# CycloneBoy/pdf_table

Hardware: AMD Instinct MI355X
Metric: pages/s (higher is better)
Workload: dtype bf16

## Files before the change

pdf_table_amd/csrc/rec_kernels.hip:

```cpp
#include <math.h>

#include "common.h"

namespace PT_FMT_NS {

typedef __attribute__((ext_vector_type(8))) __bf16 bf16x8;
typedef __attribute__((ext_vector_type(16))) float f32x16;
typedef __attribute__((ext_vector_type(4))) uint32_t u32x4;
typedef __attribute__((ext_vector_type(2))) uint32_t u32x2;

__device__ __forceinline__ float rbf2f(uint32_t bits16) { return a16_to_f32(bits16); }
__device__ __forceinline__ uint32_t rf2bf(float f) { return f32_to_a16(f); }

__global__ __launch_bounds__(256) void rec_warp_kernel(const uint8_t* __restrict__ pages, int ph, int pw,
                                                        const pt_rec_line* __restrict__ lines, int n_lines,
                                                        const long long* __restrict__ pix_off, uint8_t* __restrict__ crops) {
  a16_kernel_enter();
  const int li = blockIdx.y;
  if (li >= n_lines) return;
  const pt_rec_line L = lines[li];
  const int cw = L.crop_w, chh = L.crop_h;
  const long long npx = (long long)cw * chh;
  uint8_t* dst = crops + pix_off[li] * 3;
  const uint8_t* src = pages + (size_t)L.page * ph * pw * 3;
// ... 999 lines not shown
    __syncthreads();
    if (tid == 0) __hip_atomic_store(fl + member, s + 1, __ATOMIC_RELAXED, __HIP_MEMORY_SCOPE_AGENT);
#pragma unroll
    for (int i = 0; i < 2 * MI; ++i) {
      const int idx = tio + i * 256, m = idx >> 3, pc = idx & 7;
      const int line = line0 + m;
      if (line < B) *reinterpret_cast<u32x4*>(hout + ((size_t)line * T + t) * 512 + dir * 256 + member * 64 + pc * 8) = pv[i];
    }
  }
}

template <int MI>
static int launch_lstm_cluster(const bf16_t* gx, const bf16_t* whh, bf16_t* hout, int B, int T, int max_cl, bf16_t* hx, int* flags,
                               int* err, hipStream_t s) {
  constexpr int CLL = 64 * MI;
  constexpr int SMEM = 131072 + CLL * 72 * 2;
  static bool attr_done = false;
  if (!attr_done) {
    PT_HIP_CHECK(hipFuncSetAttribute(reinterpret_cast<const void*>(&lstm_cluster_kernel<MI>), hipFuncAttributeMaxDynamicSharedMemorySize, SMEM));
    attr_done = true;
  }
  const int nlaunch = (B + max_cl * CLL - 1) / (max_cl * CLL);
  const int per = (((B + nlaunch - 1) / nlaunch) + CLL - 1) / CLL * CLL;
  for (int b0 = 0; b0 < B; b0 += per) {
    const int nb = (B - b0) < per ? (B - b0) : per;
    const int ncl = (nb + CLL - 1) / CLL;
    PT_HIP_CHECK(hipMemsetAsync(flags, 0, (size_t)(2 * max_cl * 4) * sizeof(int), s));
    hipLaunchKernelGGL(lstm_cluster_kernel<MI>, dim3(((ncl + 7) / 8) * 32, 2), dim3(256), SMEM, s, gx + (size_t)b0 * T * 2048, whh,
                       hout + (size_t)b0 * T * 512, nb, T, ncl, hx, flags, err);
  }
  return PT_OK;
}

template <int MI, int NW>
__global__ __launch_bounds__(64 * NW, 1) void lstm_cluster8_x3_kernel(const bf16_t* __restrict__ gx, const bf16_t* __restrict__ whh,
                                                                   bf16_t* __restrict__ hout, int B, int T, int ncl,
                                                                   unsigned long long* __restrict__ hx, int* __restrict__ flags,
                                                                   int* __restrict__ err) {
  a16_kernel_enter();
  constexpr int CLL = 32 * NW * MI, NTILE = NW * MI, NTHR = 64 * NW;
  extern __shared__ __attribute__((aligned(16))) char lsm[];
  char* wl = lsm;
  constexpr int SROW = 32;
  bf16_t* stage = reinterpret_cast<bf16_t*>(lsm + 131072) + (threadIdx.x >> 6) * (2 * 32 * SROW);
  const int tid = threadIdx.x, lane = tid & 63, wave = tid >> 6;
  const int lx = lane & 31, q = lane >> 5;
  const int L = blockIdx.x, dir = blockIdx.y;
  const int member = (L >> 3) & 7, cl = (L >> 6) * 8 + (L & 7);
  if (cl >= ncl) return;
  const int line0 = cl * CLL;
  {
    for (int i = tid; i < 2 * 64 * 64; i += NTHR) {
      const int pl = i >> 12, rec = (i >> 6) & 63, ln = i & 63;
      const bf16_t* src = whh + (size_t)pl * 2 * 1024 * 256 + (size_t)dir * 1024 * 256 + (size_t)(member >> 1) * 65536 +
                          (size_t)(rec * 2 + (member & 1)) * 512 + ln * 8;
      *reinterpret_cast<u32x4*>(wl + (size_t)pl * 65536 + rec * 1024 + ln * 16) = *reinterpret_cast<const u32x4*>(src);
    }
  }
  constexpr size_t XBUF = (size_t)NTILE * 16 * 2 * 64 * 2;
  unsigned long long* hxc = hx + (size_t)(dir * ncl + cl) * 2 * XBUF;
  int* fl = flags + (dir * ncl + cl) * 8;
  float c[MI][16];
#pragma unroll
  for (int mi = 0; mi < MI; ++mi)
#pragma unroll
    for (int r = 0; r < 16; ++r) c[mi][r] = 0.f;
// ... 142 lines not shown
    PT_HIP_CHECK(hipMalloc(&e->lstm_scratch8, need));
    e->lstm_scratch8_cap = need;
  }
  unsigned long long* hx = reinterpret_cast<unsigned long long*>(e->lstm_scratch8);
  int* flags = reinterpret_cast<int*>(reinterpret_cast<char*>(e->lstm_scratch8) + (size_t)2 * max_cl * 2 * xbuf);
  int* err = nullptr;
  PT_HIP_CHECK(hipHostGetDevicePointer(reinterpret_cast<void**>(&err), e->lstm_err, 0));
  const int nlaunch = (B + max_cl * CLL - 1) / (max_cl * CLL);
  const int per = (((B + nlaunch - 1) / nlaunch) + CLL - 1) / CLL * CLL;
  for (int b0 = 0; b0 < B; b0 += per) {
    const int nb = (B - b0) < per ? (B - b0) : per;
    const int ncl = (nb + CLL - 1) / CLL;
    PT_HIP_CHECK(hipMemsetAsync(flags, 0, (size_t)(2 * max_cl * 8) * sizeof(int), s));
    hipLaunchKernelGGL((lstm_cluster8_x3_kernel<MI, NW>), dim3(((ncl + 7) / 8) * 64, 2), dim3(64 * NW), SMEM, s, gx + (size_t)b0 * T * 4096, whh,
                       hout + (size_t)b0 * T * 1024, nb, T, ncl, hx, flags, err);
  }
  return PT_OK;
}

int pt_launch_lstm(pt_engine* e, const bf16_t* gx, const bf16_t* whh, bf16_t* hout, int B, int T, int split, hipStream_t s) {
  if (B <= 0) return PT_OK;
  dim3 grid((B + 31) / 32, 2);
  static int ng2 = -1;
  if (ng2 < 0) {
    const char* ev = getenv("PT_LSTM_NG");
    ng2 = ev ? (atoi(ev) == 2) : 1;
  }
  static int use_dma = -1;
  if (use_dma < 0) {
    const char* ev = getenv("PT_LSTM_DMA");
    use_dma = ev ? atoi(ev) : 0;
  }
  if (!split && e->lstm_cluster) {
    if (!e->lstm_scratch) {
      e->lstm_max_cl = e->num_cu / 8 < 1 ? 1 : e->num_cu / 8;
      PT_HIP_CHECK(hipMalloc(&e->lstm_scratch, (size_t)2 * e->lstm_max_cl * 2 * CLL_MAX * 256 * sizeof(bf16_t) + (size_t)2 * e->lstm_max_cl * 4 * sizeof(int) + 256));
      PT_HIP_CHECK(hipHostMalloc(reinterpret_cast<void**>(&e->lstm_err), sizeof(int), hipHostMallocMapped));
      *e->lstm_err = 0;
    }
    void* scratch = e->lstm_scratch;
    int* h_err = e->lstm_err;
    const int max_cl = e->lstm_max_cl;
    if (*h_err) {
      *h_err = 0;
      e->lstm_cluster = 0;
      pt_set_error("lstm_cluster_kernel: a workgroup waited > 2^22 polls for its peers -- the launch was not co-resident "
                   "(GPU shared with another process or stream?).  Results of that call are invalid; this engine now uses "
                   "the streaming LSTM kernel: run the batch again");
      return PT_ERR_HIP;
    }
    bf16_t* hx = reinterpret_cast<bf16_t*>(scratch);
    int* flags = reinterpret_cast<int*>(reinterpret_cast<char*>(scratch) + (size_t)2 * max_cl * 2 * CLL_MAX * 256 * sizeof(bf16_t));
    int* err = nullptr;
    PT_HIP_CHECK(hipHostGetDevicePointer(reinterpret_cast<void**>(&err), h_err, 0));
    const char* ev = getenv("PT_LSTM_MI");
    const int force = ev ? atoi(ev) : 0;
    const int n2 = (B + max_cl * 128 - 1) / (max_cl * 128), n3 = (B + max_cl * 192 - 1) / (max_cl * 192);
    const bool mi3 = force == 3 || (force != 2 && n3 < n2);
    const int rc = mi3 ? launch_lstm_cluster<3>(gx, whh, hout, B, T, max_cl, hx, flags, err, s)
                       : launch_lstm_cluster<2>(gx, whh, hout, B, T, max_cl, hx, flags, err, s);
    if (rc != PT_OK) return rc;
  } else if (split == 1 && e->lstm_cluster && !(getenv("PT_LSTM_CLUSTER_X3") && atoi(getenv("PT_LSTM_CLUSTER_X3")) == 0)) {
    if (!e->lstm_err) {
      PT_HIP_CHECK(hipHostMalloc(reinterpret_cast<void**>(&e->lstm_err), sizeof(int), hipHostMallocMapped));
      *e->lstm_err = 0;
    }
    if (*e->lstm_err) {
      *e->lstm_err = 0;
      e->lstm_cluster = 0;
      pt_set_error("lstm_cluster8_x3_kernel: a workgroup waited > 2^22 polls for its peers -- the launch was not co-resident "
                   "(GPU shared with another process or stream?).  Results of that call are invalid; this engine now uses "
                   "the streaming LSTM kernel: run the batch again");
      return PT_ERR_HIP;
    }
    const int max_cl = e->num_cu / 16 < 1 ? 1 : e->num_cu / 16;
    const char* ev = getenv("PT_LSTM_MI");
    const int force = ev ? atoi(ev) : 0;
    const char* wv = getenv("PT_LSTM_X3_WAVES");
    int rc;
    if (wv && atoi(wv) == 4) {
      const int n2 = (B + max_cl * 256 - 1) / (max_cl * 256), n3 = (B + max_cl * 384 - 1) / (max_cl * 384);
      const bool mi3 = force == 3 || (force != 2 && n3 < n2);
      rc = mi3 ? launch_lstm_cluster8_x3<3, 4>(e, gx, whh, hout, B, T, s) : launch_lstm_cluster8_x3<2, 4>(e, gx, whh, hout, B, T, s);
    } else {
      const int n1 = (B + max_cl * 256 - 1) / (max_cl * 256), n2 = (B + max_cl * 512 - 1) / (max_cl * 512);
      const bool mi2 = force == 2 || (force != 1 && n2 < n1);
      rc = mi2 ? launch_lstm_cluster8_x3<2, 8>(e, gx, whh, hout, B, T, s) : launch_lstm_cluster8_x3<1, 8>(e, gx, whh, hout, B, T, s);
    }
    if (rc != PT_OK) return rc;
  } else if (split) {
    if (ng2)
      hipLaunchKernelGGL((lstm_dir_kernel<1, 2>), dim3((B + 63) / 64, 2), dim3(512), 0, s, gx, whh, hout, B, T);
    else
// ... 758 lines not shown
```

include/pdftable_hip.h:

```cpp
#ifndef PDFTABLE_HIP_H
#define PDFTABLE_HIP_H

#include <stddef.h>
#include <stdint.h>

#ifdef __cplusplus
extern "C" {
#endif

#define PT_OK 0
#define PT_ERR_INVALID 1
#define PT_ERR_HIP 2
#define PT_ERR_STATE 3
#define PT_ERR_FORMAT 4

typedef struct pt_engine pt_engine;
typedef void* pt_stream;

int pt_engine_create(int device_id, pt_engine** out);
void pt_engine_destroy(pt_engine* e);
const char* pt_last_error(void);
int pt_abi_version(void);
int pt_engine_check(pt_engine* e);
int pt_engine_set_lstm_cluster(pt_engine* e, int on);
// ... 133 lines not shown
  double minv[6];
  int32_t page, x0, y0, crop_w, crop_h, reserved;
} pt_tsr_table;

int pt_tsr_preprocess(pt_engine* e, const uint8_t* d_pages_rgb, int n_pages, int ph, int pw, const pt_tsr_table* d_tables,
                      int n, int inp_h, int inp_w, int bgr, uint16_t* d_out_bf16, pt_stream stream);

#define PT_TSR_CS_SMALL 8
#define PT_TSR_CS_FEAT 256
int pt_tsr_forward_net(pt_engine* e, const uint16_t* d_input_bf16, int n, int H, int W, float* d_hm, float* d_st,
                       float* d_wh, float* d_ax, float* d_cr, float* d_reg, pt_stream stream);

int pt_tsr_forward_net_wireless(pt_engine* e, const uint16_t* d_input_bf16, int n, int H, int W, float* d_hm, float* d_st,
                                float* d_wh, float* d_ax, float* d_cr, float* d_reg, pt_stream stream);

#define PT_TSR_MAX_CELLS 3000
int pt_tsr_decode(pt_engine* e, const float* d_hm, const float* d_st, const float* d_wh, const float* d_ax,
                  const float* d_cr, const float* d_reg, int n, int h, int w, int wiz_rev, float vis_thresh,
                  int32_t* d_counts, float* d_dets, float* d_logi, pt_stream stream);

int pt_tsr_forward_decode(pt_engine* e, const uint16_t* d_input_bf16, int n, int in_h, int in_w, int wiz_rev,
                          float vis_thresh, int32_t* d_counts, float* d_dets, float* d_logi, pt_stream stream);

int pt_tsr_process(pt_engine* e, const float* d_logi, const float* d_dets, const int32_t* h_counts, int n_tables,
                   int use_2dpe, float* d_logic, float* d_stacked, pt_stream stream);

int pt_op_conv2d(pt_engine* e, const uint16_t* d_in, int B, int H, int W, int Cin, const uint16_t* d_w_tiled,
                 const float* d_bias, int N, int ks, int stride, uint16_t* d_out, int out_cstride, int out_coff,
                 int rep, int shuffle_cout, const uint16_t* d_res, int res_mode, int relu, int split, int out_lo_off,
                 pt_stream stream);
int pt_op_conv1x1_ex(pt_engine* e, const uint16_t* d_in, int B, int H, int W, int Cin, const uint16_t* d_w_tiled, const float* d_bias,
                     int N, uint16_t* d_out, float* d_out_f32, int out_cstride, int n_valid, const float* d_res_f32, int relu,
                     const int32_t* d_ylimit, pt_stream stream);

int pt_op_dcn(pt_engine* e, const uint16_t* d_in, const float* d_om, int B, int H, int W, int C, const uint16_t* d_w_tiled,
              const float* d_bias, int N, uint16_t* d_out, int relu, int split, pt_stream stream);

int pt_op_stem7x7(pt_engine* e, const uint16_t* d_in, int B, int H, int W, const uint16_t* d_w, const float* d_bias,
                  uint16_t* d_out, int split, pt_stream stream);
int pt_op_maxpool3x3s2(pt_engine* e, const uint16_t* d_in, int B, int H, int W, int C, uint16_t* d_out, int split,
                       pt_stream stream);
int pt_op_db_head_final(pt_engine* e, const uint16_t* d_in, int B, int H, int W, const void* d_w, const float* d_bias,
                        float* d_prob, float* d_logits, int split, pt_stream stream);

int pt_op_dwconv(pt_engine* e, const uint16_t* d_in, int B, int H, int W, int C, const float* d_w_taps, const float* d_bias, int k,
                 int stride, int act, uint16_t* d_out, int split, pt_stream stream);
int pt_op_add(pt_engine* e, const uint16_t* d_a, const uint16_t* d_b, uint16_t* d_out, long long npix, int C, int split, pt_stream stream);
int pt_op_maxpool(pt_engine* e, const uint16_t* d_in, int B, int H, int W, int C, int k, int stride, int pad, uint16_t* d_out,
                  int split, pt_stream stream);
int pt_op_avgpool(pt_engine* e, const uint16_t* d_in, int B, int H, int W, int C, int k, uint16_t* d_out, int split, pt_stream stream);
int pt_op_chan_mean(pt_engine* e, const uint16_t* d_in, int B, int HW, int C, float* d_scratch, uint16_t* d_mean, int split, pt_stream stream);
int pt_op_chan_mean_scratch_floats(int B, int C);
int pt_op_scale_channels(pt_engine* e, const uint16_t* d_in, const uint16_t* d_gate, int B, int HW, int C, uint16_t* d_out,
                         int split, pt_stream stream);
int pt_op_act(pt_engine* e, const uint16_t* d_in, long long n_elems, int kind, float alpha, float beta, uint16_t* d_out, int C, int split,
              pt_stream stream);
int pt_op_copy_channels(pt_engine* e, const uint16_t* d_src, long long npix, int src_cstride, int src_coff, uint16_t* d_dst, int dst_cstride, int dst_coff,
                        int n, pt_stream stream);
int pt_op_upsample_nearest(pt_engine* e, const uint16_t* d_in, int B, int H, int W, int C, int factor, uint16_t* d_out, pt_stream stream);
int pt_op_mul(pt_engine* e, const uint16_t* d_a, const uint16_t* d_b, uint16_t* d_out, long long n_elems, int C, int split, pt_stream stream);
int pt_copy_bytes(pt_engine* e, const void* src, void* dst, long long nbytes, pt_stream stream);
int pt_op_layernorm(pt_engine* e, const uint16_t* d_in, long long rows, int c_pad, int c, const float* d_gamma, const float* d_beta, float eps,
                    uint16_t* d_out, int split, pt_stream stream);
int pt_op_softmax(pt_engine* e, const uint16_t* d_in, long long rows, int c_pad, int c, float* d_out_f32, uint16_t* d_out_bf16, int split, pt_stream stream);
int pt_op_attention(pt_engine* e, const uint16_t* d_qkv, int B, int T, int heads, int d, int qkv_cstride, float scale, uint16_t* d_out, int out_cstride,
                    int split, pt_stream stream);
// ... 47 lines not shown
```

pdf_table_amd/csrc/c_api.hip:

```cpp
#include <stdarg.h>
#include <stdio.h>
#include <stdlib.h>

#include <cmath>

#include "common.h"

namespace PT_FMT_NS {
namespace api {

static int ensure(void** buf, size_t* cap, size_t need);

int pt_engine_check(pt_engine* e) {
  PT_REQUIRE(e, "pt_engine_check: null engine");
  if (e->lstm_err && *e->lstm_err) {
    *e->lstm_err = 0;
    e->lstm_cluster = 0;
    pt_set_error("lstm_cluster_kernel: a workgroup waited > 2^22 polls for its peers -- the launch was not co-resident "
                 "(GPU shared with another process or stream?).  The recognition results since the last check are invalid; "
                 "this engine now uses the streaming LSTM kernel (pt_engine_set_lstm_cluster(e, 0)): run the batch again");
    return PT_ERR_HIP;
  }
  return PT_OK;
}
// ... 886 lines not shown
      if (rc != PT_OK) return rc;
    }
    rc = pt_pplcnet_forward_net(e, slot, xin, nb, out_h, out_w, textline, d_logits + (size_t)i0 * PT_CLS_MAX_CLASSES, n_classes, s,
                                PT_ARENA_CLS);
    if (rc != PT_OK) return rc;
  }
  return PT_OK;
}

int pt_op_conv2d(pt_engine* e, const uint16_t* d_in, int B, int H, int W, int Cin, const uint16_t* d_w_tiled,
                 const float* d_bias, int N, int ks, int stride, uint16_t* d_out, int out_cstride, int out_coff,
                 int rep, int shuffle_cout, const uint16_t* d_res, int res_mode, int relu, int split, int out_lo_off,
                 pt_stream stream) {
  PT_REQUIRE(e != nullptr, "pt_op_conv2d: null engine");
  ConvDesc d;
  d.in = d_in; d.B = B; d.H = H; d.W = W; d.Cin = Cin; d.w = d_w_tiled; d.bias = d_bias; d.N = N; d.ks = ks;
  d.stride = stride; d.out = d_out; d.out_cstride = out_cstride; d.out_coff = out_coff; d.rep = rep;
  d.shuffle_cout = shuffle_cout; d.res = d_res; d.res_mode = res_mode; d.relu = relu;
  d.split = split; d.out_lo_off = out_lo_off;
  return pt_launch_conv(e, d, reinterpret_cast<hipStream_t>(stream));
}

int pt_op_conv1x1_ex(pt_engine* e, const uint16_t* d_in, int B, int H, int W, int Cin, const uint16_t* d_w_tiled, const float* d_bias,
                     int N, uint16_t* d_out, float* d_out_f32, int out_cstride, int n_valid, const float* d_res_f32, int relu,
                     const int32_t* d_ylimit, pt_stream stream) {
  PT_REQUIRE(e != nullptr, "pt_op_conv1x1_ex: null engine");
  ConvDesc d;
  d.in = d_in; d.B = B; d.H = H; d.W = W; d.Cin = Cin; d.w = d_w_tiled; d.bias = d_bias; d.N = N; d.ks = 1; d.stride = 1;
  d.out = d_out_f32 ? nullptr : d_out; d.out_f32 = d_out_f32; d.out_cstride = out_cstride; d.n_valid = n_valid; d.res_f32 = d_res_f32;
  d.relu = relu; d.ylimit = d_ylimit;
  return pt_launch_conv(e, d, reinterpret_cast<hipStream_t>(stream));
}

int pt_op_stem7x7(pt_engine* e, const uint16_t* d_in, int B, int H, int W, const uint16_t* d_w, const float* d_bias,
                  uint16_t* d_out, int split, pt_stream stream) {
  PT_REQUIRE(e != nullptr, "pt_op_stem7x7: null engine");
  return pt_launch_stem7x7(e, d_in, B, H, W, d_w, d_bias, d_out, split, reinterpret_cast<hipStream_t>(stream));
}

int pt_op_maxpool3x3s2(pt_engine* e, const uint16_t* d_in, int B, int H, int W, int C, uint16_t* d_out, int split,
                       pt_stream stream) {
  PT_REQUIRE(e && d_in && d_out, "pt_op_maxpool3x3s2: bad arguments");
  return pt_launch_maxpool3x3s2(d_in, B, H, W, C, d_out, split, reinterpret_cast<hipStream_t>(stream));
}

int pt_op_db_head_final(pt_engine* e, const uint16_t* d_in, int B, int H, int W, const void* d_w, const float* d_bias,
                        float* d_prob, float* d_logits, int split, pt_stream stream) {
  PT_REQUIRE(e && d_in && d_w && d_bias && (d_prob || d_logits), "pt_op_db_head_final: bad arguments");
  return pt_launch_db_head_final(d_in, B, H, W, d_w, d_bias, d_prob, d_logits, split, reinterpret_cast<hipStream_t>(stream));
}

int pt_op_dcn(pt_engine* e, const uint16_t* d_in, const float* d_om, int B, int H, int W, int C, const uint16_t* d_w_tiled,
              const float* d_bias, int N, uint16_t* d_out, int relu, int split, pt_stream stream) {
  PT_REQUIRE(e && d_in && d_om && d_w_tiled && d_bias && d_out, "pt_op_dcn: null argument");
  PT_REQUIRE(B > 0 && H > 0 && W > 0, "pt_op_dcn: empty map (B=%d H=%d W=%d)", B, H, W);
  return pt_launch_dcn_fused(e, d_in, d_om, d_w_tiled, d_bias, d_out, B, H, W, C, N, split, relu, reinterpret_cast<hipStream_t>(stream));
}

int pt_profile_enable(pt_engine* e, int on) {
  PT_REQUIRE(e != nullptr, "pt_profile_enable: null engine");
  PT_REQUIRE(on >= 0 && on < 2 + PT_PROF_NCLASS, "pt_profile_enable: mode %d out of range", on);
  if (on && !e->prof.h_lims)
    PT_HIP_CHECK(hipHostMalloc(reinterpret_cast<void**>(&e->prof.h_lims), PtProfile::MAX_LIMS * sizeof(int), hipHostMallocDefault));
  e->prof.on = on;
  return PT_OK;
}
// ... 76 lines not shown
```

pdf_table_amd/engine.py:

```python
from __future__ import annotations

import contextlib
import ctypes as C
import functools
import threading
from typing import Optional, Sequence, Tuple

import numpy as np
import torch

from . import lib as L

__all__ = ["HipEngine", "REC_LINE_DTYPE", "CLS_IMAGE_DTYPE", "REC_PP_ITEM_DTYPE"]

TSR_TABLE_DTYPE = np.dtype([("minv", "<f8", (6,)), ("page", "<i4"), ("x0", "<i4"), ("y0", "<i4"),
                            ("crop_w", "<i4"), ("crop_h", "<i4"), ("reserved", "<i4")])
CLS_IMAGE_DTYPE = np.dtype([("offset", "<i8"), ("h", "<i4"), ("w", "<i4")])
REC_LINE_DTYPE = np.dtype([("minv", np.float64, (9,)), ("page", np.int32), ("crop_w", np.int32), ("crop_h", np.int32),
                           ("reserved", np.int32)])


REC_PP_ITEM_DTYPE = np.dtype([("line", "<i4"), ("resized_w", "<i4"), ("img_w", "<i4"), ("reserved", "<i4"),
                              ("out_off", "<i8")])

# ... 537 lines not shown
                  shuffle_cout: int = 0, out: Optional[torch.Tensor] = None, out_coff: int = 0,
                  split: int = 0) -> torch.Tensor:
        self._chk(x, self.act_dtype, "x")
        self._chk(bias, torch.float32, "bias")
        B, H, W, Cin = x.shape
        m = 2 if split else 1
        Cin //= m
        N = bias.numel()
        pad = ks // 2
        Ho, Wo = (H + 2 * pad - ks) // stride + 1, (W + 2 * pad - ks) // stride + 1
        if out is None:
            if shuffle_cout:
                out = torch.empty((B, 2 * Ho, 2 * Wo, shuffle_cout * m), dtype=self.act_dtype, device=self._tdev)
            else:
                out = torch.empty((B, Ho * rep, Wo * rep, N * m), dtype=self.act_dtype, device=self._tdev)
        L.check(self.lib.pt_op_conv2d(self._h, _ptr(x), B, H, W, Cin, _ptr(w_tiled), _ptr(bias), N, ks, stride,
                                      _ptr(out), out.shape[-1], out_coff, rep, shuffle_cout, _ptr(res), res_mode,
                                      int(relu), int(split), out.shape[-1] // 2, self._stream()), "pt_op_conv2d")
        return out

    def op_conv1x1_ex(self, x: torch.Tensor, w_tiled: torch.Tensor, bias: torch.Tensor, relu: int = 0, out_f32: bool = False,
                      n_valid: int = 0, res_f32: Optional[torch.Tensor] = None, ylimit: Optional[torch.Tensor] = None) -> torch.Tensor:
        self._chk(x, self.act_dtype, "x")
        self._chk(bias, torch.float32, "bias")
        B, H, W, Cin = x.shape
        N = bias.numel()
        cs = n_valid or N
        out = torch.zeros((B, H, W, cs), dtype=torch.float32 if out_f32 else self.act_dtype, device=self._tdev)
        L.check(self.lib.pt_op_conv1x1_ex(self._h, _ptr(x), B, H, W, Cin, _ptr(w_tiled), _ptr(bias), N, None if out_f32 else _ptr(out),
                                          _ptr(out) if out_f32 else None, cs, n_valid, _ptr(res_f32), int(relu), _ptr(ylimit),
                                          self._stream()), "pt_op_conv1x1_ex")
        return out

    def op_dcn(self, x: torch.Tensor, om: torch.Tensor, w_tiled: torch.Tensor, bias: torch.Tensor, relu: bool = True, split: int = 0) -> torch.Tensor:
        self._chk(x, self.act_dtype, "x")
        self._chk(om, torch.float32, "om")
        self._chk(bias, torch.float32, "bias")
        B, H, W, Cc = x.shape
        m = 2 if split else 1
        Cc //= m
        if tuple(om.shape) != (B, H, W, 32):
            raise ValueError(f"op_dcn: om must be [B,H,W,32], got {tuple(om.shape)}")
        N = bias.numel()
        out = torch.empty((B, H, W, N * m), dtype=self.act_dtype, device=self._tdev)
        L.check(self.lib.pt_op_dcn(self._h, _ptr(x), _ptr(om), B, H, W, Cc, _ptr(w_tiled), _ptr(bias), N, _ptr(out), int(relu), int(split),
                                   self._stream()), "pt_op_dcn")
        return out

    def op_dwconv(self, x: torch.Tensor, w_taps: torch.Tensor, bias: torch.Tensor, k: int, stride: int = 1, act: int = 0, split: bool = False) -> torch.Tensor:
        self._chk(x, self.act_dtype, "x")
        self._chk(w_taps, torch.float32, "w_taps")
        self._chk(bias, torch.float32, "bias")
        B, H, W, Cc = x.shape
        pad = k // 2
        out = torch.empty((B, (H + 2 * pad - k) // stride + 1, (W + 2 * pad - k) // stride + 1, Cc), dtype=self.act_dtype, device=self._tdev)
        L.check(self.lib.pt_op_dwconv(self._h, _ptr(x), B, H, W, Cc // 2 if split else Cc, _ptr(w_taps), _ptr(bias), k, stride, act, _ptr(out), int(split),
                                      self._stream()), "pt_op_dwconv")
        return out

    def op_add(self, a: torch.Tensor, b: torch.Tensor, split: bool = False) -> torch.Tensor:
        self._chk(a, self.act_dtype, "a")
        self._chk(b, self.act_dtype, "b")
        if a.shape != b.shape:
            raise ValueError(f"op_add: shapes differ: {tuple(a.shape)} vs {tuple(b.shape)}")
        out = torch.empty_like(a)
        L.check(self.lib.pt_op_add(self._h, _ptr(a), _ptr(b), _ptr(out), a.numel() // a.shape[-1], a.shape[-1] // 2 if split else a.shape[-1], int(split),
# ... 227 lines not shown
```

pdf_table_amd/lib.py:

```python
from __future__ import annotations

import ctypes as C
import os

_HERE = os.path.dirname(os.path.abspath(__file__))
LIB_PATH = os.environ.get("PT_LIB_PATH") or os.path.join(_HERE, "libpdftable_hip.so")

PT_MODEL_DB_RESNET18 = 1
PT_MODEL_CRNN = 2
PT_MODEL_LORE_DLA34 = 3
PT_MODEL_LORE_PROCESSOR = 4
PT_MODEL_PICODET = 5
PT_MODEL_LORE_RESNET18 = 6
PT_MODEL_DB_NAS = 7
PT_MODEL_PPLCNET = 8
PT_MODEL_CONVNEXT_VIT = 16
PT_MODEL_MTL_BACKBONE = 17
PT_MODEL_MTL_DECODER = 18
PT_CVIT_W, PT_CVIT_CHUNK_W, PT_CVIT_CHUNK_STEP, PT_CVIT_T, PT_CVIT_NCLS = 804, 300, 252, 201, 7644
PT_CLS_SLOTS = 4
PT_CLS_MAX_CLASSES = 16
PT_LAYOUT_HEAD_CS, PT_LAYOUT_CAND_FLOATS = 40, 48
PT_DET_PRE_DB_PP = 0
PT_DET_PRE_DB_TORCH = 1
# ... 46 lines not shown
        "pt_rec_forward_net": (i, [vp, vp, i, vp, vp, vp]),
        "pt_rec_preprocess": (i, [vp, vp, i, i, i, vp, vp, i, vp, vp]),
        "pt_rec_cvit_forward": (i, [vp, vp, i, i, i, vp, vp, vp, i, vp, vp, vp]),
        "pt_rec_cvit_forward_crops": (i, [vp, vp, vp, vp, vp, i, vp, vp, vp]),
        "pt_rec_cvit_forward_net": (i, [vp, vp, i, i, vp, vp, vp, vp]),
        "pt_rec_cvit_preprocess_crops": (i, [vp, vp, vp, vp, i, vp, vp]),
        "pt_tsr_mtl_backbone_net": (i, [vp, vp, i, i, i, vp, vp]),
        "pt_tsr_mtl_preprocess": (i, [vp, vp, i, i, i, vp, i, i, vp, vp]),
        "pt_tsr_mtl_resized_size": (None, [i, i, i, ip, ip]),
        "pt_tsr_mtl_decoder_config": (i, [vp, ip]),
        "pt_tsr_mtl_structure": (i, [vp, vp, i, i, vp, vp, ip, ip, i, vp]),
        "pt_tsr_mtl_cells": (i, [vp, i, vp, vp, vp, ip, i, vp]),
        "pt_rec_pp_preprocess": (i, [vp, vp, i, i, i, vp, vp, i, vp, i, i, i, vp, vp]),
        "pt_rec_pp_preprocess_crops": (i, [vp, vp, vp, vp, i, vp, i, i, i, vp, vp]),
        "pt_layout_plan": (i, [i, i, ip, ip]),
        "pt_layout_preprocess": (i, [vp, vp, i, i, i, i, i, vp, vp]),
        "pt_layout_forward_net": (i, [vp, vp, i, i, i, vp, vp, vp, vp, vp]),
        "pt_layout_candidates": (i, [vp, vp, vp, vp, vp, i, i, i, i, f, i, vp, vp, vp]),
        "pt_layout_forward": (i, [vp, vp, i, i, i, i, i, i, f, i, vp, vp, vp]),
        "pt_tsr_preprocess": (i, [vp, vp, i, i, i, vp, i, i, i, i, vp, vp]),
        "pt_tsr_forward_net": (i, [vp, vp, i, i, i, vp, vp, vp, vp, vp, vp, vp]),
        "pt_tsr_forward_net_wireless": (i, [vp, vp, i, i, i, vp, vp, vp, vp, vp, vp, vp]),
        "pt_tsr_decode": (i, [vp, vp, vp, vp, vp, vp, vp, i, i, i, i, f, vp, vp, vp, vp]),
        "pt_tsr_forward_decode": (i, [vp, vp, i, i, i, i, f, vp, vp, vp, vp]),
        "pt_tsr_process": (i, [vp, vp, vp, vp, i, i, vp, vp, vp]),
        "pt_hard_nms": (i, [vp, vp, vp, i, C.c_double, i, vp, vp]),
        "pt_cls_preprocess": (i, [vp, vp, vp, i, i, i, i, i, vp, vp]),
        "pt_cls_forward_net": (i, [vp, i, vp, i, i, i, i, vp, ip, vp]),
        "pt_cls_forward": (i, [vp, i, vp, vp, i, i, i, i, i, i, vp, ip, vp]),
        "pt_cls_forward_lines": (i, [vp, i, vp, i, i, i, vp, vp, i, i, i, i, i, i, vp, ip, vp]),
        "pt_cls_forward_lines_direct": (i, [vp, i, vp, i, i, i, vp, i, i, i, i, i, i, vp, ip, vp]),
        "pt_op_conv2d": (i, [vp, vp, i, i, i, i, vp, vp, i, i, i, vp, i, i, i, i, vp, i, i, i, i, vp]),
        "pt_op_conv1x1_ex": (i, [vp, vp, i, i, i, i, vp, vp, i, vp, vp, i, i, vp, i, vp, vp]),
        "pt_op_dcn": (i, [vp, vp, vp, i, i, i, i, vp, vp, i, vp, i, i, vp]),
        "pt_op_stem7x7": (i, [vp, vp, i, i, i, vp, vp, vp, i, vp]),
        "pt_op_maxpool3x3s2": (i, [vp, vp, i, i, i, i, vp, i, vp]),
        "pt_op_db_head_final": (i, [vp, vp, i, i, i, vp, vp, vp, vp, i, vp]),
        "pt_op_dwconv": (i, [vp, vp, i, i, i, i, vp, vp, i, i, i, vp, i, vp]),
        "pt_op_add": (i, [vp, vp, vp, vp, C.c_longlong, i, i, vp]),
        "pt_op_maxpool": (i, [vp, vp, i, i, i, i, i, i, i, vp, i, vp]),
        "pt_op_avgpool": (i, [vp, vp, i, i, i, i, i, vp, i, vp]),
        "pt_op_chan_mean": (i, [vp, vp, i, i, i, vp, vp, i, vp]),
        "pt_op_chan_mean_scratch_floats": (i, [i, i]),
        "pt_op_scale_channels": (i, [vp, vp, vp, i, i, i, vp, i, vp]),
        "pt_op_act": (i, [vp, vp, C.c_longlong, i, C.c_float, C.c_float, vp, i, i, vp]),
        "pt_op_copy_channels": (i, [vp, vp, C.c_longlong, i, i, vp, i, i, i, vp]),
        "pt_op_upsample_nearest": (i, [vp, vp, i, i, i, i, i, vp, vp]),
        "pt_op_mul": (i, [vp, vp, vp, vp, C.c_longlong, i, i, vp]),
        "pt_copy_bytes": (i, [vp, vp, vp, C.c_longlong, vp]),
        "pt_op_layernorm": (i, [vp, vp, C.c_longlong, i, i, vp, vp, C.c_float, vp, i, vp]),
        "pt_op_softmax": (i, [vp, vp, C.c_longlong, i, i, vp, vp, i, vp]),
        "pt_op_attention": (i, [vp, vp, i, i, i, i, i, C.c_float, vp, i, i, vp]),
        "pt_profile_enable": (i, [vp, i]),
        "pt_profile_read": (i, [vp, vp, vp, vp]),
        "pt_profile_read_labels": (i, [vp, C.c_char_p, i]),
    }
    for name, (res, args) in P.items():
        fn = getattr(lib, name)
        fn.restype = res
        fn.argtypes = args
    return P


EXPORTS = None


# ... 22 lines not shown
```

Measured before the change: 795.9.

## Add multi-wave-per-tile LSTM cluster kernel and make it the default path

```diff
diff --git a/pdf_table_amd/csrc/rec_kernels.hip b/pdf_table_amd/csrc/rec_kernels.hip
--- a/pdf_table_amd/csrc/rec_kernels.hip
+++ b/pdf_table_amd/csrc/rec_kernels.hip
@@ -1055,6 +1055,170 @@
   return PT_OK;
 }
 
+template <int MI>
+__global__ __launch_bounds__(256 * MI, 1) void lstm_cluster_mw_kernel(const bf16_t* __restrict__ gx, const bf16_t* __restrict__ whh,
+                                                                      bf16_t* __restrict__ hout, int B, int T, int ncl,
+                                                                      bf16_t* __restrict__ hx, int* __restrict__ flags,
+                                                                      int* __restrict__ err) {
+  a16_kernel_enter();
+  constexpr int CLL = 64 * MI, NT = 256 * MI;
+  extern __shared__ __attribute__((aligned(16))) char lsm[];
+  char* wl = lsm;
+  constexpr int SROW = 72;
+  bf16_t* stage = reinterpret_cast<bf16_t*>(lsm + 131072);
+  const int tid = threadIdx.x, lane = tid & 63, wave = tid >> 6;
+  const int lx = lane & 31, q = lane >> 5;
+  const int L = blockIdx.x, dir = blockIdx.y;
+  const int member = (L >> 3) & 3, cl = (L >> 5) * 8 + (L & 7);
+  if (cl >= ncl) return;
+  const int line0 = cl * CLL;
+  const int h = wave & 1, tile = wave >> 1;
+  if (wave < 4) __builtin_amdgcn_s_setprio(MI - 1);
+  else if (MI == 3 && wave < 8) __builtin_amdgcn_s_setprio(1);
+  {
+    const u32x4* src = reinterpret_cast<const u32x4*>(whh + (size_t)dir * 1024 * 256 + (size_t)member * 65536);
+    for (int i = tid; i < 8192; i += NT) reinterpret_cast<u32x4*>(wl)[i] = src[i];
+  }
+  unsigned long long* hxc = reinterpret_cast<unsigned long long*>(hx + (size_t)(dir * ncl + cl) * 2 * (CLL * 256));
+  int* fl = flags + (dir * ncl + cl) * 4;
+  float c[16];
+#pragma unroll
+  for (int r = 0; r < 16; ++r) c[r] = 0.f;
+  bool dead = false;
+  __syncthreads();
+  for (int s = 0; s < T; ++s) {
+    const int t = dir ? T - 1 - s : s;
+    u32x2 gv[16];
+    int last = B - 1;
+    asm volatile("" : "+v"(last));
+    const bf16_t* gxt = gx + (size_t)t * 2048 + dir * 1024 + (member * 64 + h * 32 + lx) * 4;
+#pragma unroll
+    for (int r = 0; r < 16; ++r) {
+      const int line = line0 + tile * 32 + (r & 3) + 8 * (r >> 2) + 4 * q;
+      const int lc = line < last ? line : last;
+      gv[r] = *reinterpret_cast<const u32x2*>(gxt + (size_t)lc * T * 2048);
+    }
+    if (s > 0 && !(PT_CL_ABL & 4)) {
+      if (tid < 4 && !dead) {
+        int spins = 0;
+        while (__hip_atomic_load(fl + tid, __ATOMIC_RELAXED, __HIP_MEMORY_SCOPE_AGENT) < s) {
+          if (++spins > (1 << 22)) { dead = true; __hip_atomic_store(err, 1, __ATOMIC_RELAXED, __HIP_MEMORY_SCOPE_SYSTEM); break; }
+          __builtin_amdgcn_s_sleep(1);
+        }
+      }
+      __syncthreads();
+    }
+    f32x16 acc[4];
+#pragma unroll
+    for (int g = 0; g < 4; ++g)
+#pragma unroll
+      for (int r = 0; r < 16; ++r) acc[g][r] = 0.f;
+    if (s > 0 && !(PT_CL_ABL & 1)) {
+      const unsigned long long* hp = hxc + (size_t)((s - 1) & 1) * (CLL * 256 / 4);
+      asm volatile("" : "+s"(hp));
+      constexpr int NH = MI == 3 ? 4 : 1, KH = 16 / NH;
+      bf16x8 wf[4];
+#pragma unroll
+      for (int g = 0; g < 4; ++g) wf[g] = *reinterpret_cast<const bf16x8*>(wl + (g * 2 + h) * 1024 + lane * 16);
+#pragma unroll
+      for (int hh = 0; hh < NH; ++hh) {
+        unsigned long long af[KH][2];
+#pragma unroll
+        for (int kk = 0; kk < KH; ++kk) {
+          const gptr_u64 pp = (gptr_u64)hp + ((size_t)(tile * 16 + hh * KH + kk) * 64 + lane) * 2;
+          af[kk][0] = __hip_atomic_load(pp, __ATOMIC_RELAXED, __HIP_MEMORY_SCOPE_AGENT);
+          af[kk][1] = __hip_atomic_load(pp + 1, __ATOMIC_RELAXED, __HIP_MEMORY_SCOPE_AGENT);
+        }
+#pragma unroll
+        for (int kk = 0; kk < KH; ++kk) {
+          const int ks = hh * KH + kk;
+          const unsigned long long two[2] = {af[kk][0], af[kk][1]};
+          const bf16x8 a = __builtin_bit_cast(bf16x8, two);
+#pragma unroll
+          for (int g = 0; g < 4; ++g) {
+            acc[g] = mfma_32x32x16_a16(a, wf[g], acc[g]);
+            if (ks + 1 < 16) wf[g] = *reinterpret_cast<const bf16x8*>(wl + (((ks + 1) * 4 + g) * 2 + h) * 1024 + lane * 16);
+          }
+        }
+        __builtin_amdgcn_sched_group_barrier(0x020, 2 * KH, 0);
+        if (hh == 0) __builtin_amdgcn_sched_group_barrier(0x100, 4, 0);
+#pragma unroll
+        for (int kk = 0; kk < KH; ++kk)
+#pragma unroll
+          for (int g = 0; g < 4; ++g) {
+            __builtin_amdgcn_sched_group_barrier(0x008, 1, 0);
+            if (hh * KH + kk + 1 < 16) __builtin_amdgcn_sched_group_barrier(0x100, 1, 0);
+          }
+        __builtin_amdgcn_sched_barrier(0);
+      }
+    }
+#pragma unroll
+    for (int r = 0; r < 16; ++r) {
+      const int m = tile * 32 + (r & 3) + 8 * (r >> 2) + 4 * q;
+      const float gi = acc[0][r] + rbf2f(gv[r].x & 0xFFFFu);
+      const float gf = acc[1][r] + rbf2f(gv[r].x >> 16);
+      const float gg = acc[2][r] + rbf2f(gv[r].y & 0xFFFFu);
+      const float go = acc[3][r] + rbf2f(gv[r].y >> 16);
+#if PT_CL_ABL & 2
+      const float si = gi * 0.25f, sf = gf * 0.25f, so = go * 0.25f;
+      const float cn = sf * c[r] + si * gg;
+      c[r] = cn;
+      stage[m * SROW + h * 32 + lx] = (bf16_t)rf2bf(so * cn);
+#else
+      const float si = fast_sigmoid(gi), sf = fast_sigmoid(gf), so = fast_sigmoid(go);
+      const float cn = sf * c[r] + si * fast_tanh(gg);
+      c[r] = cn;
+      stage[m * SROW + h * 32 + lx] = (bf16_t)rf2bf(so * fast_tanh(cn));
+#endif
+    }
+    __syncthreads();
+    unsigned long long* hw = hxc + (size_t)(s & 1) * (CLL * 256 / 4);
+    int tio = tid;
+    asm volatile("" : "+v"(tio));
+    u32x4 pv[2];
+#pragma unroll
+    for (int i = 0; i < 2; ++i) {
+      const int idx = tio + i * NT, m = idx >> 3, pc = idx & 7;
+      pv[i] = *reinterpret_cast<const u32x4*>(stage + m * SROW + pc * 8);
+      const int ks = 4 * member + (pc >> 1), qq = pc & 1;
+      unsigned long long* dp = hw + ((size_t)((m >> 5) * 16 + ks) * 64 + qq * 32 + (m & 31)) * 2;
+      __hip_atomic_store(dp, (unsigned long long)pv[i].x | ((unsigned long long)pv[i].y << 32), __ATOMIC_RELAXED, __HIP_MEMORY_SCOPE_AGENT);
+      __hip_atomic_store(dp + 1, (unsigned long long)pv[i].z | ((unsigned long long)pv[i].w << 32), __ATOMIC_RELAXED, __HIP_MEMORY_SCOPE_AGENT);
+    }
+    asm volatile("s_waitcnt vmcnt(0)" ::: "memory");
+    __syncthreads();
+    if (tid == 0) __hip_atomic_store(fl + member, s + 1, __ATOMIC_RELAXED, __HIP_MEMORY_SCOPE_AGENT);
+#pragma unroll
+    for (int i = 0; i < 2; ++i) {
+      const int idx = tio + i * NT, m = idx >> 3, pc = idx & 7;
+      const int line = line0 + m;
+      if (line < B) *reinterpret_cast<u32x4*>(hout + ((size_t)line * T + t) * 512 + dir * 256 + member * 64 + pc * 8) = pv[i];
+    }
+  }
+}
+
+template <int MI>
+static int launch_lstm_cluster_mw(const bf16_t* gx, const bf16_t* whh, bf16_t* hout, int B, int T, int max_cl, bf16_t* hx, int* flags,
+                                  int* err, hipStream_t s) {
+  constexpr int CLL = 64 * MI;
+  constexpr int SMEM = 131072 + CLL * 72 * 2;
+  static bool attr_done = false;
+  if (!attr_done) {
+    PT_HIP_CHECK(hipFuncSetAttribute(reinterpret_cast<const void*>(&lstm_cluster_mw_kernel<MI>), hipFuncAttributeMaxDynamicSharedMemorySize, SMEM));
+    attr_done = true;
+  }
+  const int nlaunch = (B + max_cl * CLL - 1) / (max_cl * CLL);
+  const int per = (((B + nlaunch - 1) / nlaunch) + CLL - 1) / CLL * CLL;
+  for (int b0 = 0; b0 < B; b0 += per) {
+    const int nb = (B - b0) < per ? (B - b0) : per;
+    const int ncl = (nb + CLL - 1) / CLL;
+    PT_HIP_CHECK(hipMemsetAsync(flags, 0, (size_t)(2 * max_cl * 4) * sizeof(int), s));
+    hipLaunchKernelGGL(lstm_cluster_mw_kernel<MI>, dim3(((ncl + 7) / 8) * 32, 2), dim3(256 * MI), SMEM, s, gx + (size_t)b0 * T * 2048, whh,
+                       hout + (size_t)b0 * T * 512, nb, T, ncl, hx, flags, err);
+  }
+  return PT_OK;
+}
+
 template <int MI, int NW>
 __global__ __launch_bounds__(64 * NW, 1) void lstm_cluster8_x3_kernel(const bf16_t* __restrict__ gx, const bf16_t* __restrict__ whh,
                                                                    bf16_t* __restrict__ hout, int B, int T, int ncl,
@@ -1288,8 +1452,14 @@
     const int force = ev ? atoi(ev) : 0;
     const int n2 = (B + max_cl * 128 - 1) / (max_cl * 128), n3 = (B + max_cl * 192 - 1) / (max_cl * 192);
     const bool mi3 = force == 3 || (force != 2 && n3 < n2);
-    const int rc = mi3 ? launch_lstm_cluster<3>(gx, whh, hout, B, T, max_cl, hx, flags, err, s)
-                       : launch_lstm_cluster<2>(gx, whh, hout, B, T, max_cl, hx, flags, err, s);
+    const char* mw = getenv("PT_LSTM_CLUSTER_MW");
+    int rc;
+    if (mw && atoi(mw) == 0)
+      rc = mi3 ? launch_lstm_cluster<3>(gx, whh, hout, B, T, max_cl, hx, flags, err, s)
+               : launch_lstm_cluster<2>(gx, whh, hout, B, T, max_cl, hx, flags, err, s);
+    else
+      rc = mi3 ? launch_lstm_cluster_mw<3>(gx, whh, hout, B, T, max_cl, hx, flags, err, s)
+               : launch_lstm_cluster_mw<2>(gx, whh, hout, B, T, max_cl, hx, flags, err, s);
     if (rc != PT_OK) return rc;
   } else if (split == 1 && e->lstm_cluster && !(getenv("PT_LSTM_CLUSTER_X3") && atoi(getenv("PT_LSTM_CLUSTER_X3")) == 0)) {
     if (!e->lstm_err) {
```

New measurement: 800.1, median of 6. No clear change (+0.5%).

## Add 8-workgroup cluster LSTM kernel splitting hidden units across cooperating blocks

Applied to the files above, without the earlier changes.

```diff
diff --git a/include/pdftable_hip.h b/include/pdftable_hip.h
--- a/include/pdftable_hip.h
+++ b/include/pdftable_hip.h
@@ -189,6 +189,8 @@
 int pt_op_conv1x1_ex(pt_engine* e, const uint16_t* d_in, int B, int H, int W, int Cin, const uint16_t* d_w_tiled, const float* d_bias,
                      int N, uint16_t* d_out, float* d_out_f32, int out_cstride, int n_valid, const float* d_res_f32, int relu,
                      const int32_t* d_ylimit, pt_stream stream);
+
+int pt_op_lstm(pt_engine* e, const uint16_t* d_gx, const uint16_t* d_whh, uint16_t* d_hout, int B, int T, pt_stream stream);
 
 int pt_op_dcn(pt_engine* e, const uint16_t* d_in, const float* d_om, int B, int H, int W, int C, const uint16_t* d_w_tiled,
               const float* d_bias, int N, uint16_t* d_out, int relu, int split, pt_stream stream);
diff --git a/pdf_table_amd/csrc/c_api.hip b/pdf_table_amd/csrc/c_api.hip
--- a/pdf_table_amd/csrc/c_api.hip
+++ b/pdf_table_amd/csrc/c_api.hip
@@ -942,6 +942,12 @@
   return pt_launch_conv(e, d, reinterpret_cast<hipStream_t>(stream));
 }
 
+int pt_op_lstm(pt_engine* e, const uint16_t* d_gx, const uint16_t* d_whh, uint16_t* d_hout, int B, int T, pt_stream stream) {
+  PT_REQUIRE(e && d_gx && d_whh && d_hout && B >= 0 && T > 0, "pt_op_lstm: bad arguments");
+  PT_REQUIRE(e->precision == PT_PRECISION_BF16 || e->precision == PT_PRECISION_F16, "pt_op_lstm: single-pass precision only");
+  return pt_launch_lstm(e, d_gx, d_whh, d_hout, B, T, 0, reinterpret_cast<hipStream_t>(stream));
+}
+
 int pt_op_stem7x7(pt_engine* e, const uint16_t* d_in, int B, int H, int W, const uint16_t* d_w, const float* d_bias,
                   uint16_t* d_out, int split, pt_stream stream) {
   PT_REQUIRE(e != nullptr, "pt_op_stem7x7: null engine");
diff --git a/pdf_table_amd/csrc/rec_kernels.hip b/pdf_table_amd/csrc/rec_kernels.hip
--- a/pdf_table_amd/csrc/rec_kernels.hip
+++ b/pdf_table_amd/csrc/rec_kernels.hip
@@ -1055,6 +1055,211 @@
   return PT_OK;
 }
 
+template <int NW, int MI>
+__global__ __launch_bounds__(64 * NW, 8 / NW) void lstm_cluster8_kernel(const bf16_t* __restrict__ gx, const bf16_t* __restrict__ whh,
+                                                                       bf16_t* __restrict__ hout, int B, int T, int ncl, int ntile,
+                                                                       unsigned long long* __restrict__ hx, int* __restrict__ flags,
+                                                                       int* __restrict__ err) {
+  a16_kernel_enter();
+  constexpr int NTHR = 64 * NW, SROW = 32;
+  extern __shared__ __attribute__((aligned(16))) char lsm[];
+  char* wl = lsm;
+  bf16_t* stage = reinterpret_cast<bf16_t*>(lsm + 65536) + (threadIdx.x >> 6) * (MI * 32 * SROW);
+  const int tid = threadIdx.x, lane = tid & 63, wave = tid >> 6;
+  const int lx = lane & 31, q = lane >> 5;
+  const int L = blockIdx.x, dir = blockIdx.y;
+  const int member = (L >> 3) & 7, cl = (L >> 6) * 8 + (L & 7);
+  if (cl >= ncl) return;
+  const int line0 = cl * 32 * ntile;
+  {
+    const bf16_t* src = whh + (size_t)dir * 1024 * 256 + (size_t)(member >> 1) * 65536 + (member & 1) * 512;
+    for (int i = tid; i < 64 * 64; i += NTHR) {
+      const int rec = i >> 6, ln = i & 63;
+      *reinterpret_cast<u32x4*>(wl + rec * 1024 + ln * 16) = *reinterpret_cast<const u32x4*>(src + (size_t)rec * 1024 + ln * 8);
+    }
+  }
+  const size_t xbuf = (size_t)ntile * 16 * 64 * 2;
+  unsigned long long* hxc = hx + (size_t)(dir * ncl + cl) * 2 * xbuf;
+  int* fl = flags + (dir * ncl + cl) * 8;
+  float c[MI][16];
+#pragma unroll
+  for (int mi = 0; mi < MI; ++mi)
+#pragma unroll
+    for (int r = 0; r < 16; ++r) c[mi][r] = 0.f;
+  bool dead = false;
+  __syncthreads();
+  for (int s = 0; s < T; ++s) {
+    const int t = dir ? T - 1 - s : s;
+    int last = B - 1;
+    asm volatile("" : "+v"(last));
+    const bf16_t* gxt = gx + (size_t)t * 2048 + dir * 1024 + (member * 32 + lx) * 4;
+    u32x2 gv[MI][16];
+#pragma unroll
+    for (int mi = 0; mi < MI; ++mi)
+#pragma unroll
+      for (int r = 0; r < 16; ++r) {
+        const int line = line0 + (wave + NW * mi) * 32 + (r & 3) + 8 * (r >> 2) + 4 * q;
+        const int lc = line < last ? line : last;
+        gv[mi][r] = *reinterpret_cast<const u32x2*>(gxt + (size_t)lc * T * 2048);
+      }
+    if (s > 0) {
+      if (tid < 8 && !dead) {
+        int spins = 0;
+        while (__hip_atomic_load(fl + tid, __ATOMIC_RELAXED, __HIP_MEMORY_SCOPE_AGENT) < s) {
+          if (++spins > (1 << 22)) { dead = true; __hip_atomic_store(err, 1, __ATOMIC_RELAXED, __HIP_MEMORY_SCOPE_SYSTEM); break; }
+          __builtin_amdgcn_s_sleep(1);
+        }
+      }
+      __syncthreads();
+    }
+    const unsigned long long* hp = hxc + (size_t)((s - 1) & 1) * xbuf;
+    unsigned long long* hw = hxc + (size_t)(s & 1) * xbuf;
+    asm volatile("" : "+s"(hp), "+s"(hw));
+    unsigned long long af[8][2];
+    auto fetch = [&](int tile, int k0) {
+#pragma unroll
+      for (int ks = 0; ks < 8; ++ks) {
+        const gptr_u64 pp = (gptr_u64)hp + ((size_t)(tile * 16 + k0 + ks) * 64 + lane) * 2;
+        af[ks][0] = __hip_atomic_load(pp, __ATOMIC_RELAXED, __HIP_MEMORY_SCOPE_AGENT);
+        af[ks][1] = __hip_atomic_load(pp + 1, __ATOMIC_RELAXED, __HIP_MEMORY_SCOPE_AGENT);
+      }
+    };
+    if (s > 0 && wave < ntile) fetch(wave, 0);
+#pragma unroll
+    for (int mi = 0; mi < MI; ++mi) {
+      const int tile = wave + NW * mi;
+      if (tile >= ntile) break;
+      f32x16 acc[4];
+#pragma unroll
+      for (int g = 0; g < 4; ++g)
+#pragma unroll
+        for (int r = 0; r < 16; ++r) acc[g][r] = 0.f;
+      if (s > 0) {
+#pragma unroll
+        for (int k0 = 0; k0 < 16; k0 += 8) {
+          if (k0 == 8) fetch(tile, 8);
+          bf16x8 wf[4];
+#pragma unroll
+          for (int g = 0; g < 4; ++g) wf[g] = *reinterpret_cast<const bf16x8*>(wl + (k0 * 4 + g) * 1024 + lane * 16);
+#pragma unroll
+          for (int ks = 0; ks < 8; ++ks) {
+            const unsigned long long two[2] = {af[ks][0], af[ks][1]};
+            const bf16x8 a = __builtin_bit_cast(bf16x8, two);
+#pragma unroll
+            for (int g = 0; g < 4; ++g) {
+              acc[g] = mfma_32x32x16_a16(a, wf[g], acc[g]);
+              if (ks + 1 < 8) wf[g] = *reinterpret_cast<const bf16x8*>(wl + ((k0 + ks + 1) * 4 + g) * 1024 + lane * 16);
+            }
+          }
+          if (k0 == 8) __builtin_amdgcn_sched_group_barrier(0x020, 16, 0);
+          __builtin_amdgcn_sched_group_barrier(0x100, 4, 0);
+#pragma unroll
+          for (int ks = 0; ks < 8; ++ks)
+#pragma unroll
+            for (int g = 0; g < 4; ++g) {
+              __builtin_amdgcn_sched_group_barrier(0x008, 1, 0);
+              if (ks + 1 < 8) __builtin_amdgcn_sched_group_barrier(0x100, 1, 0);
+            }
+          __builtin_amdgcn_sched_barrier(0);
+        }
+        if (mi + 1 < MI && tile + NW < ntile) fetch(tile + NW, 0);
+        __builtin_amdgcn_sched_barrier(0);
+      }
+      bf16_t* st = stage + mi * 32 * SROW;
+#pragma unroll
+      for (int r = 0; r < 16; ++r) {
+        const float gi = acc[0][r] + rbf2f(gv[mi][r].x & 0xFFFFu);
+        const float gf = acc[1][r] + rbf2f(gv[mi][r].x >> 16);
+        const float gg = acc[2][r] + rbf2f(gv[mi][r].y & 0xFFFFu);
+        const float go = acc[3][r] + rbf2f(gv[mi][r].y >> 16);
+        const float si = fast_sigmoid(gi), sf = fast_sigmoid(gf), so = fast_sigmoid(go);
+        const float cn = sf * c[mi][r] + si * fast_tanh(gg);
+        c[mi][r] = cn;
+        st[((r & 3) + 8 * (r >> 2) + 4 * q) * SROW + lx] = (bf16_t)rf2bf(so * fast_tanh(cn));
+      }
+#pragma unroll
+      for (int i = 0; i < 2; ++i) {
+        const int idx = lane + i * 64, ml = idx >> 2, pc = idx & 3;
+        const u32x4 pv = *reinterpret_cast<const u32x4*>(st + ml * SROW + pc * 8);
+        __attribute__((address_space(1))) unsigned long long* dp =
+            (__attribute__((address_space(1))) unsigned long long*)hw + ((size_t)(tile * 16 + 2 * member + (pc >> 1)) * 64 + (pc & 1) * 32 + ml) * 2;
+        __hip_atomic_store(dp, (unsigned long long)pv.x | ((unsigned long long)pv.y << 32), __ATOMIC_RELAXED, __HIP_MEMORY_SCOPE_AGENT);
+        __hip_atomic_store(dp + 1, (unsigned long long)pv.z | ((unsigned long long)pv.w << 32), __ATOMIC_RELAXED, __HIP_MEMORY_SCOPE_AGENT);
+      }
+      __builtin_amdgcn_sched_barrier(0);
+    }
+    asm volatile("s_waitcnt vmcnt(0)" ::: "memory");
+    __syncthreads();
+    if (tid == 0) __hip_atomic_store(fl + member, s + 1, __ATOMIC_RELAXED, __HIP_MEMORY_SCOPE_AGENT);
+#pragma unroll
+    for (int mi = 0; mi < MI; ++mi) {
+      const int tile = wave + NW * mi;
+      if (tile >= ntile) break;
+#pragma unroll
+      for (int i = 0; i < 2; ++i) {
+        const int idx = lane + i * 64, ml = idx >> 2, pc = idx & 3;
+        const int line = line0 + tile * 32 + ml;
+        const u32x4 pv = *reinterpret_cast<const u32x4*>(stage + (mi * 32 + ml) * SROW + pc * 8);
+        if (line < B) *reinterpret_cast<u32x4*>(hout + ((size_t)line * T + t) * 512 + dir * 256 + member * 32 + pc * 8) = pv;
+      }
+    }
+  }
+}
+
+template <int NW, int MI>
+static int lstm_cluster8_max_cl(pt_engine* e, int smem, int* max_cl) {
+  static int occ = -1;
+  if (occ < 0) {
+    int nb = 0;
+    PT_HIP_CHECK(hipOccupancyMaxActiveBlocksPerMultiprocessor(&nb, reinterpret_cast<const void*>(&lstm_cluster8_kernel<NW, MI>), 64 * NW, smem));
+    occ = nb;
+  }
+  const int slots = occ * (e->num_cu / 8);
+  const int per_xcd = (slots - slots / 8) / 16;
+  *max_cl = 8 * (per_xcd < 1 ? 1 : per_xcd);
+  return PT_OK;
+}
+
+template <int NW, int MI>
+static int launch_lstm_cluster8(pt_engine* e, const bf16_t* gx, const bf16_t* whh, bf16_t* hout, int B, int T, int* err, hipStream_t s) {
+  constexpr int SMEM = 65536 + NW * MI * 32 * 32 * 2;
+  static_assert(SMEM <= 163840, "LDS");
+  static bool attr_done = false;
+  if (!attr_done) {
+    PT_HIP_CHECK(hipFuncSetAttribute(reinterpret_cast<const void*>(&lstm_cluster8_kernel<NW, MI>), hipFuncAttributeMaxDynamicSharedMemorySize, SMEM));
+    attr_done = true;
+  }
+  int max_cl = 0;
+  const int rc = lstm_cluster8_max_cl<NW, MI>(e, SMEM, &max_cl);
+  if (rc != PT_OK) return rc;
+  constexpr int TMAX = NW * MI;
+  const size_t xbuf = (size_t)TMAX * 16 * 64 * 2 * sizeof(unsigned long long);
+  const size_t need = (size_t)2 * max_cl * 2 * xbuf + (size_t)2 * max_cl * 8 * sizeof(int) + 256;
+  if (need > e->lstm_scratch8_cap) {
+    PT_HIP_CHECK(hipStreamSynchronize(s));
+    if (e->lstm_scratch8) PT_HIP_CHECK(hipFree(e->lstm_scratch8));
+    e->lstm_scratch8 = nullptr; e->lstm_scratch8_cap = 0;
+    PT_HIP_CHECK(hipMalloc(&e->lstm_scratch8, need));
+    e->lstm_scratch8_cap = need;
+  }
+  unsigned long long* hx = reinterpret_cast<unsigned long long*>(e->lstm_scratch8);
+  int* flags = reinterpret_cast<int*>(reinterpret_cast<char*>(e->lstm_scratch8) + (size_t)2 * max_cl * 2 * xbuf);
+  const int nlaunch = (B + max_cl * TMAX * 32 - 1) / (max_cl * TMAX * 32);
+  const int per = (B + nlaunch - 1) / nlaunch;
+  int ntile = (per + max_cl * 32 - 1) / (max_cl * 32);
+  const char* ev = getenv("PT_LSTM_C8_TILES");
+  if (ev && atoi(ev) >= ntile && atoi(ev) <= TMAX) ntile = atoi(ev);
+  const int cll = 32 * ntile;
+  for (int b0 = 0; b0 < B; b0 += per) {
+    const int nb = (B - b0) < per ? (B - b0) : per;
+    const int ncl = (nb + cll - 1) / cll;
+    PT_HIP_CHECK(hipMemsetAsync(flags, 0, (size_t)(2 * max_cl * 8) * sizeof(int), s));
+    hipLaunchKernelGGL((lstm_cluster8_kernel<NW, MI>), dim3(((ncl + 7) / 8) * 64, 2), dim3(64 * NW), SMEM, s, gx + (size_t)b0 * T * 2048, whh,
+                       hout + (size_t)b0 * T * 512, nb, T, ncl, ntile, hx, flags, err);
+  }
+  return PT_OK;
+}
+
 template <int MI, int NW>
 __global__ __launch_bounds__(64 * NW, 1) void lstm_cluster8_x3_kernel(const bf16_t* __restrict__ gx, const bf16_t* __restrict__ whh,
                                                                    bf16_t* __restrict__ hout, int B, int T, int ncl,
@@ -1263,15 +1468,11 @@
     use_dma = ev ? atoi(ev) : 0;
   }
   if (!split && e->lstm_cluster) {
-    if (!e->lstm_scratch) {
-      e->lstm_max_cl = e->num_cu / 8 < 1 ? 1 : e->num_cu / 8;
-      PT_HIP_CHECK(hipMalloc(&e->lstm_scratch, (size_t)2 * e->lstm_max_cl * 2 * CLL_MAX * 256 * sizeof(bf16_t) + (size_t)2 * e->lstm_max_cl * 4 * sizeof(int) + 256));
+    if (!e->lstm_err) {
       PT_HIP_CHECK(hipHostMalloc(reinterpret_cast<void**>(&e->lstm_err), sizeof(int), hipHostMallocMapped));
       *e->lstm_err = 0;
     }
-    void* scratch = e->lstm_scratch;
     int* h_err = e->lstm_err;
-    const int max_cl = e->lstm_max_cl;
     if (*h_err) {
       *h_err = 0;
       e->lstm_cluster = 0;
@@ -1280,10 +1481,25 @@
                    "the streaming LSTM kernel: run the batch again");
       return PT_ERR_HIP;
     }
+    int* err = nullptr;
+    PT_HIP_CHECK(hipHostGetDevicePointer(reinterpret_cast<void**>(&err), h_err, 0));
+    const char* c8 = getenv("PT_LSTM_CLUSTER8");
+    if (!(c8 && atoi(c8) == 0)) {
+      const char* wv = getenv("PT_LSTM_C8_WAVES");
+      const int rc = (wv && atoi(wv) == 8) ? launch_lstm_cluster8<8, 2>(e, gx, whh, hout, B, T, err, s)
+                                           : launch_lstm_cluster8<4, 2>(e, gx, whh, hout, B, T, err, s);
+      if (rc != PT_OK) return rc;
+      PT_HIP_CHECK(hipGetLastError());
+      return PT_OK;
+    }
+    if (!e->lstm_scratch) {
+      e->lstm_max_cl = e->num_cu / 8 < 1 ? 1 : e->num_cu / 8;
+      PT_HIP_CHECK(hipMalloc(&e->lstm_scratch, (size_t)2 * e->lstm_max_cl * 2 * CLL_MAX * 256 * sizeof(bf16_t) + (size_t)2 * e->lstm_max_cl * 4 * sizeof(int) + 256));
+    }
+    void* scratch = e->lstm_scratch;
+    const int max_cl = e->lstm_max_cl;
     bf16_t* hx = reinterpret_cast<bf16_t*>(scratch);
     int* flags = reinterpret_cast<int*>(reinterpret_cast<char*>(scratch) + (size_t)2 * max_cl * 2 * CLL_MAX * 256 * sizeof(bf16_t));
-    int* err = nullptr;
-    PT_HIP_CHECK(hipHostGetDevicePointer(reinterpret_cast<void**>(&err), h_err, 0));
     const char* ev = getenv("PT_LSTM_MI");
     const int force = ev ? atoi(ev) : 0;
     const int n2 = (B + max_cl * 128 - 1) / (max_cl * 128), n3 = (B + max_cl * 192 - 1) / (max_cl * 192);
diff --git a/pdf_table_amd/engine.py b/pdf_table_amd/engine.py
--- a/pdf_table_amd/engine.py
+++ b/pdf_table_amd/engine.py
@@ -593,6 +593,13 @@
                                           self._stream()), "pt_op_conv1x1_ex")
         return out
 
+    def op_lstm(self, gx: torch.Tensor, whh: torch.Tensor) -> torch.Tensor:
+        self._chk(gx, self.act_dtype, "gx")
+        B, T, _ = gx.shape
+        out = torch.zeros((B, T, 512), dtype=self.act_dtype, device=self._tdev)
+        L.check(self.lib.pt_op_lstm(self._h, _ptr(gx), _ptr(whh), _ptr(out), B, T, self._stream()), "pt_op_lstm")
+        return out
+
     def op_dcn(self, x: torch.Tensor, om: torch.Tensor, w_tiled: torch.Tensor, bias: torch.Tensor, relu: bool = True, split: int = 0) -> torch.Tensor:
         self._chk(x, self.act_dtype, "x")
         self._chk(om, torch.float32, "om")
diff --git a/pdf_table_amd/lib.py b/pdf_table_amd/lib.py
--- a/pdf_table_amd/lib.py
+++ b/pdf_table_amd/lib.py
@@ -102,6 +102,7 @@
         "pt_cls_forward_lines_direct": (i, [vp, i, vp, i, i, i, vp, i, i, i, i, i, i, vp, ip, vp]),
         "pt_op_conv2d": (i, [vp, vp, i, i, i, i, vp, vp, i, i, i, vp, i, i, i, i, vp, i, i, i, i, vp]),
         "pt_op_conv1x1_ex": (i, [vp, vp, i, i, i, i, vp, vp, i, vp, vp, i, i, vp, i, vp, vp]),
+        "pt_op_lstm": (i, [vp, vp, vp, vp, i, i, vp]),
         "pt_op_dcn": (i, [vp, vp, vp, i, i, i, i, vp, vp, i, vp, i, i, vp]),
         "pt_op_stem7x7": (i, [vp, vp, i, i, i, vp, vp, vp, i, vp]),
         "pt_op_maxpool3x3s2": (i, [vp, vp, i, i, i, i, vp, i, vp]),
```

Result: no change. 813.6 before, 817.0 after, median of 6 (+0.4%).
